# PatrickHwang/Explicit-tf2-Recommendation

Hardware: AMD Instinct MI355X
Metric: examples/sec fwd+bwd, DeepFM 10M-vocab x16d batch 8192 (higher is better)
Workload: dtype f32; 1 GPU; DeepFM fwd+bwd, 26 categorical fields, 10M-vocab x 16d, batch 8192 (BASELINE.json metric); vocab=10000000, fields=26, embedding_dims=16, batch_per_gpu=8192, id_distribution=uniform, parallelism=single GPU, global_batch=8192, hipgraph=one graph per 5 steps, 32 resident batches

## Files before the change

### explicit-tf2-recommendation_amd/csrc/deepfm_fused.hip

```cpp
#include "deepfm_fused.h"
#include <math.h>

namespace {

constexpr int LD = 32;

struct ReduceArgs {
  const float* dK0part; const float* small; int nwg; int D; int64_t B;
  float* dK0; float* dK1; float* db0; float* db1; float* dK2; float* db2; float* dbias; float* loss;
};

constexpr int RC = 16;
constexpr int RS = 64;
__host__ __device__ inline int reduce_blocks(int D) {
  return (int)(((int64_t)D * U1 / 4 + RC - 1) / RC) + (SMALL / 4 + RC - 1) / RC;
}

__device__ __forceinline__ void reduce_body(const ReduceArgs& r, int bidx) {
  const float* __restrict__ dK0part = r.dK0part;
  const float* __restrict__ small = r.small;
  const int nwg = r.nwg, D = r.D;
  const int64_t B = r.B;
  float* __restrict__ dK0 = r.dK0; float* __restrict__ dK1 = r.dK1; float* __restrict__ db0 = r.db0;
  float* __restrict__ db1 = r.db1; float* __restrict__ dK2 = r.dK2; float* __restrict__ db2 = r.db2;
  float* __restrict__ dbias = r.dbias; float* __restrict__ loss = r.loss;
  __shared__ float4 red[RS][RC];
  __shared__ float4 red2[8][RC];
  const int lane = threadIdx.x & (RC - 1), q = threadIdx.x / RC;
  const int64_t n0 = (int64_t)D * U1;
  const int nb0 = (int)((n0 / 4 + RC - 1) / RC);
  float4 acc = make_float4(0.f, 0.f, 0.f, 0.f);
  int64_t e4 = 0;
  const bool is_small = bidx >= nb0;
  const float* src;
  int64_t stride;
  bool in = false;
  if (!is_small) {
    e4 = (int64_t)bidx * RC + lane;
    in = e4 * 4 < n0;
    src = dK0part + e4 * 4;
    stride = n0;
  } else {
    e4 = (int64_t)(bidx - nb0) * RC + lane;
    in = e4 * 4 < SMALL;
    src = small + e4 * 4;
    stride = SMALL;
  }
  if (in) {
    int w = q;
    for (; w + 3 * RS < nwg; w += 4 * RS) {
      float4 x[4];
#pragma unroll
      for (int j = 0; j < 4; ++j) x[j] = *reinterpret_cast<const float4*>(src + (int64_t)(w + RS * j) * stride);
#pragma unroll
      for (int j = 0; j < 4; ++j) { acc.x += x[j].x; acc.y += x[j].y; acc.z += x[j].z; acc.w += x[j].w; }
    }
    for (; w < nwg; w += RS) {
      float4 x = *reinterpret_cast<const float4*>(src + (int64_t)w * stride);
      acc.x += x.x; acc.y += x.y; acc.z += x.z; acc.w += x.w;
    }
  }
  red[q][lane] = acc;
  __syncthreads();
  if (q < 8) {
    float4 s = red[8 * q][lane];
#pragma unroll
    for (int k = 1; k < 8; ++k) {
      float4 x = red[8 * q + k][lane];
      s.x += x.x; s.y += x.y; s.z += x.z; s.w += x.w;
    }
    red2[q][lane] = s;
  }
  __syncthreads();
  if (q != 0) return;
  float4 s = red2[0][lane];
#pragma unroll
  for (int k = 1; k < 8; ++k) {
    float4 x = red2[k][lane];
    s.x += x.x; s.y += x.y; s.z += x.z; s.w += x.w;
  }
  if (!is_small) {
    if (e4 * 4 < n0) *reinterpret_cast<float4*>(dK0 + e4 * 4) = s;
    return;
  }
  if (e4 * 4 >= SMALL) return;
  float sv[4] = {s.x, s.y, s.z, s.w};
#pragma unroll
  for (int i = 0; i < 4; ++i) {
    int k = (int)(e4 * 4) + i;
    if (k < SM_DB0) dK1[k - SM_DK1] = sv[i];
    else if (k < SM_DB1) db0[k - SM_DB0] = sv[i];
    else if (k < SM_DK2) db1[k - SM_DB1] = sv[i];
    else if (k < SM_DB2) dK2[k - SM_DK2] = sv[i];
    else if (k == SM_DB2) { db2[0] = sv[i]; dbias[0] = sv[i]; }
    else if (k == SM_LOSS) loss[0] = sv[i] / (float)B;
  }
}

struct ColSegArgs {
  const float4* vals; const float* gz; const int32_t* perm; const int64_t* col_uid; const int32_t* col_seg;
  const int32_t* col_nu; int64_t B; int F; int64_t* uniq_ids; float4* g_embed; float* g_w; int64_t* n_uniq; int packed;
  float* table; float* m_e; float* v_e; float* m_w; float* v_w; int64_t V; float lr_t, b1, b2, eps;
  const int32_t* slot_map;
  const float* lr_t_dev;
  int64_t ldm, ldw;
  int32_t* last; const int64_t* step_dev;
};

__device__ __forceinline__ void adam_chunk(const ColSegArgs& k, int64_t id, int c, const float4& g) {
  float4* vp = reinterpret_cast<float4*>(k.table + id * LD) + c;
  float4* mp = reinterpret_cast<float4*>(k.m_e + id * k.ldm) + c;
  float4* qp = reinterpret_cast<float4*>(k.v_e + id * k.ldm) + c;
  float4 x = *vp, m = *mp, v = *qp;
  adam_touch(x.x, m.x, v.x, g.x, k.lr_t, k.b1, k.b2, k.eps);
  adam_touch(x.y, m.y, v.y, g.y, k.lr_t, k.b1, k.b2, k.eps);
  adam_touch(x.z, m.z, v.z, g.z, k.lr_t, k.b1, k.b2, k.eps);
  adam_touch(x.w, m.w, v.w, g.w, k.lr_t, k.b1, k.b2, k.eps);
  *vp = x; *mp = m; *qp = v;
}
__device__ __forceinline__ void adam_w(const ColSegArgs& k, int64_t id, float g) {
  float x = k.table[id * LD + E16], m = k.m_w[id * k.ldw], v = k.v_w[id * k.ldw];
  adam_touch(x, m, v, g, k.lr_t, k.b1, k.b2, k.eps);
  k.table[id * LD + E16] = x; k.m_w[id * k.ldw] = m; k.v_w[id * k.ldw] = v;
}

__device__ __forceinline__ void colseg_body(const ColSegArgs& k, int bidx) {
  const float4* __restrict__ vals = k.vals;
  const float* __restrict__ gz = k.gz;
  const int32_t* __restrict__ perm = k.perm;
  const int64_t* __restrict__ col_uid = k.col_uid;
  const int32_t* __restrict__ col_seg = k.col_seg;
  const int32_t* __restrict__ col_nu = k.col_nu;
  const int64_t B = k.B;
  const int F = k.F;
  int64_t* __restrict__ uniq_ids = k.uniq_ids;
  float4* __restrict__ g_embed = k.g_embed;
  float* __restrict__ g_w = k.g_w;
  int64_t* __restrict__ n_uniq = k.n_uniq;
  const int packed = k.packed;
  const int tid = threadIdx.x, lane = tid & 63;
  const int c = tid & 3;
  const int64_t grp = ((int64_t)bidx * blockDim.x + tid) >> 2;
  const int f = (int)(grp / B);
  int u = (int)(grp - (int64_t)f * B);
  if ((B & 63) == 0) {
    const int w = u >> 4, g = u & 15;
    u = (g >> 2) * (int)(B >> 2) + 4 * w + (g & 3);
  }
  const bool in_range = f < F;
  __shared__ int nu_s[REC_MAX_COLS];
  if (tid < F) nu_s[tid] = col_nu[tid];
  __syncthreads();
  int64_t before = 0, total = 0;
  for (int q = 0; q < F; ++q) {
    int nq = nu_s[q];
    if (q < f) before += nq;
    total += nq;
  }
  const int nu = in_range ? nu_s[f] : 0;
  const bool live = in_range && u < nu;
  int s0 = 0, s1 = 0;
  if (live) {
    s0 = col_seg[(int64_t)f * (B + 1) + u];
    s1 = col_seg[(int64_t)f * (B + 1) + u + 1];
  }
  float4 acc = make_float4(0.f, 0.f, 0.f, 0.f);
  float accw = 0.f;
  const int32_t* pf = perm + (int64_t)f * B;
  int s_end = s1 < s0 + 16 ? s1 : s0 + 16;
  for (int s = s0; s < s_end; ++s) {
    int64_t b = pf[s];
    float4 x = vals[(b * F + f) * 4 + c];
    acc.x += x.x; acc.y += x.y; acc.z += x.z; acc.w += x.w;
    accw += gz[b];
  }
  unsigned long long longm = __ballot(live && (s1 - s0) > 16 && c == 0);
  while (longm) {
    int src = __ffsll((long long)longm) - 1;
    longm &= longm - 1;
    int rs0 = __shfl(s0, src, 64) + 16, rs1 = __shfl(s1, src, 64);
    int rf = __shfl(f, src, 64);
    const int32_t* rp = perm + (int64_t)rf * B;
    float4 pa = make_float4(0.f, 0.f, 0.f, 0.f);
    float pw = 0.f;
#pragma unroll 4
    for (int s = rs0 + (lane >> 2); s < rs1; s += 16) {
      int64_t b = rp[s];
      float4 x = vals[(b * F + rf) * 4 + c];
      pa.x += x.x; pa.y += x.y; pa.z += x.z; pa.w += x.w;
      pw += gz[b];
    }
#pragma unroll
    for (int o = 4; o < 64; o <<= 1) {
      pa.x += __shfl_xor(pa.x, o, 64); pa.y += __shfl_xor(pa.y, o, 64);
      pa.z += __shfl_xor(pa.z, o, 64); pa.w += __shfl_xor(pa.w, o, 64);
      pw += __shfl_xor(pw, o, 64);
    }
    if ((lane & ~3) == src) {
      acc.x += pa.x; acc.y += pa.y; acc.z += pa.z; acc.w += pa.w;
      accw += pw;
    }
  }
  if (!in_range) return;
  int64_t dst;
  int64_t idv;
  if (live) {
    dst = before + u;
    idv = col_uid[(int64_t)f * B + u];
    if (k.slot_map) dst = k.slot_map[dst];
  } else {
    if (k.slot_map) return;
    dst = total + ((int64_t)f * B - before) + (u - nu);
    idv = col_uid[0];
    acc = make_float4(0.f, 0.f, 0.f, 0.f);
    accw = 0.f;
  }
  if (packed) {
    g_embed[dst * 5 + c] = acc;
    if (c == 0) g_embed[dst * 5 + 4] = make_float4(accw, 0.f, 0.f, 0.f);
  } else {
    g_embed[dst * 4 + c] = acc;
    if (c == 0) g_w[dst] = accw;
  }
  if (c == 0 && uniq_ids) uniq_ids[dst] = idv;
  if (grp == 0 && c == 0 && n_uniq) *n_uniq = total;
}


constexpr int FIX_T = 1024, FIX_HUGE = 128, FIX_SHORT = 17, FIX_SKEW = 256;
__device__ __forceinline__ int fix_deal(int t, int64_t B) {
  if ((B & 63) != 0) return t;
  return ((t & 63) >> 2) * (int)(B >> 4) + 4 * (t >> 6) + (t & 3);
}
__device__ __forceinline__ int fix_spread(int t, int64_t B) {
  if ((B & 63) != 0) return t;
  return (t & 63) * (int)(B >> 6) + (t >> 6);
}
__device__ __forceinline__ int fix_group_src(unsigned long long mask, int lane) {
  int src = -1;
  const int g = lane >> 2;
  for (int i = 0; i < 16 && mask; ++i) {
    const int sl = __ffsll((long long)mask) - 1;
    mask &= mask - 1;
    if (g == i) src = sl;
  }
  return src;
}
__device__ __forceinline__ void fixup_body(const ColSegArgs& k_in, int bidx) {
  ColSegArgs k = k_in;
  if (k.lr_t_dev) k.lr_t = *k.lr_t_dev;
  const float4* __restrict__ vals = k.vals;
  const float* __restrict__ gz = k.gz;
  const int64_t B = k.B;
  const int F = k.F;
  float4* __restrict__ g_embed = k.g_embed;
  const int tid = threadIdx.x, lane = tid & 63;
  const int per_col = (int)((B + FIX_T - 1) / FIX_T);
  const int f = bidx / per_col;
  const int t = (bidx - f * per_col) * FIX_T + tid;
  const int u = fix_deal(t, B);
  __shared__ int nu_s[REC_MAX_COLS];
  __shared__ int huge_n, huge_s0[128], huge_s1[128], huge_u[128];
  __shared__ float huge_gz[128];
  __shared__ float4 hpart[FIX_T / 64][4];
  __shared__ float hw_s[FIX_T / 64];
  if (tid < F) nu_s[tid] = k.col_nu[tid];
  if (tid == 0) huge_n = 0;
  __syncthreads();
  int64_t before = 0, total = 0;
  for (int q = 0; q < F; ++q) {
    const int nq = nu_s[q];
    if (q < f) before += nq;
    total += nq;
  }
  const int nu = nu_s[f];
  const bool in_col = t < B;
  const bool live = in_col && u < nu;
  const int32_t* pf = k.perm + (int64_t)f * B;
  int s0 = 0, s1 = 0;
  if (live) {
    s0 = k.col_seg[(int64_t)f * (B + 1) + u];
    s1 = k.col_seg[(int64_t)f * (B + 1) + u + 1];
  }
  const int len = s1 - s0;
  const int64_t dst = before + u;
  const bool adam = k.table != nullptr;
  float accw = 0.f;
  if (live) {
    accw = gz[pf[s0]];
    const int64_t id = k.col_uid[(int64_t)f * B + u];
    if (len == 2) {
      const int64_t b2 = pf[s0 + 1];
      const float4* r2 = vals + (b2 * F + f) * 4;
      float4 a0 = g_embed[dst * 4], a1 = g_embed[dst * 4 + 1], a2 = g_embed[dst * 4 + 2], a3 = g_embed[dst * 4 + 3];
      const float4 x0 = r2[0], x1 = r2[1], x2 = r2[2], x3 = r2[3];
      a0.x += x0.x; a0.y += x0.y; a0.z += x0.z; a0.w += x0.w;
      a1.x += x1.x; a1.y += x1.y; a1.z += x1.z; a1.w += x1.w;
      a2.x += x2.x; a2.y += x2.y; a2.z += x2.z; a2.w += x2.w;
      a3.x += x3.x; a3.y += x3.y; a3.z += x3.z; a3.w += x3.w;
      g_embed[dst * 4] = a0; g_embed[dst * 4 + 1] = a1; g_embed[dst * 4 + 2] = a2; g_embed[dst * 4 + 3] = a3;
      k.g_w[dst] = accw + gz[b2];
    }
    if (len == 1) k.g_w[dst] = accw;
    k.uniq_ids[dst] = id;
  } else if (in_col) {
    const int64_t d2 = total + ((int64_t)f * B - before) + (u - nu);
    const float4 z = make_float4(0.f, 0.f, 0.f, 0.f);
    g_embed[d2 * 4] = z; g_embed[d2 * 4 + 1] = z; g_embed[d2 * 4 + 2] = z; g_embed[d2 * 4 + 3] = z;
    k.g_w[d2] = 0.f;
    k.uniq_ids[d2] = k.col_uid[0];
  }
  const bool skew = B - nu > FIX_SKEW;
  const int ub = skew ? fix_spread(t, B) : u;
  int s0b = s0, s1b = s1;
  if (skew) {
    s0b = 0; s1b = 0;
    if (in_col && ub < nu) {
      s0b = k.col_seg[(int64_t)f * (B + 1) + ub];
      s1b = k.col_seg[(int64_t)f * (B + 1) + ub + 1];
    }
  }
  const int lenb = s1b - s0b;
  float accwb = 0.f;
  if (lenb > 2) accwb = skew ? gz[pf[s0b]] : accw;
  if (skew && lenb > FIX_HUGE) {
    const int i = atomicAdd(&huge_n, 1);
    if (i < 128) { huge_s0[i] = s0b; huge_s1[i] = s1b; huge_u[i] = ub; huge_gz[i] = accwb; }
  }
  const int r = lane >> 2, c = lane & 3;
  {
    unsigned long long shortm = __ballot(skew && lenb > 2 && lenb <= FIX_SHORT);
#ifdef ABL_NOSHORT
    shortm = 0;
#endif
    while (shortm) {
      const int src = fix_group_src(shortm, lane);
      const bool has = src >= 0;
      const int sl = has ? src : 0;
      const int gs0 = __shfl(s0b, sl, 64), gs1_ = __shfl(s1b, sl, 64), gu = __shfl(ub, sl, 64);
      float wsum = __shfl(accwb, sl, 64);
      const int gs1 = has ? gs1_ : 0;
      const int64_t gdst = before + gu;
      float4 acc = make_float4(0.f, 0.f, 0.f, 0.f);
      if (has) acc = g_embed[gdst * 4 + c];
      for (int sp = gs0 + 1; __any(sp < gs1); sp += 4) {
        if (sp < gs1) {
          int e[4];
#pragma unroll
          for (int j = 0; j < 4; ++j) e[j] = pf[sp + j < gs1 ? sp + j : gs1 - 1];
          float4 xm[4];
          float gm[4];
#pragma unroll
          for (int j = 0; j < 4; ++j) {
            xm[j] = vals[((int64_t)e[j] * F + f) * 4 + c];
            gm[j] = gz[e[j]];
          }
#pragma unroll
          for (int j = 0; j < 4; ++j) {
            if (sp + j < gs1) {
              acc.x += xm[j].x; acc.y += xm[j].y; acc.z += xm[j].z; acc.w += xm[j].w;
              wsum += gm[j];
            }
          }
        }
      }
      if (has) {
        g_embed[gdst * 4 + c] = acc;
        if (c == 0) k.g_w[gdst] = wsum;
      }
      for (int i = 0; i < 16 && shortm; ++i) shortm &= shortm - 1;
    }
  }
  unsigned long long longm = __ballot(skew ? (lenb > FIX_SHORT && lenb <= FIX_HUGE) : lenb > 2);
#ifdef ABL_NOLONG
  longm = 0;
#endif
  while (longm) {
    const int src = __ffsll((long long)longm) - 1;
    longm &= longm - 1;
    const int rs0 = __shfl(s0b, src, 64), rs1 = __shfl(s1b, src, 64);
    const int ru = __shfl(ub, src, 64);
    const float rgz = __shfl(accwb, src, 64);
    const int64_t rdst = before + ru;
    float4 pa = make_float4(0.f, 0.f, 0.f, 0.f);
    float pw = 0.f;
#pragma unroll 4
    for (int s = rs0 + 1 + r; s < rs1; s += 16) {
      const int64_t b = pf[s];
      const float4 x = vals[(b * F + f) * 4 + c];
      pa.x += x.x; pa.y += x.y; pa.z += x.z; pa.w += x.w;
      pw += gz[b];
    }
#pragma unroll
    for (int o = 4; o < 64; o <<= 1) {
      pa.x += __shfl_xor(pa.x, o, 64); pa.y += __shfl_xor(pa.y, o, 64);
      pa.z += __shfl_xor(pa.z, o, 64); pa.w += __shfl_xor(pa.w, o, 64);
      pw += __shfl_xor(pw, o, 64);
    }
    if (r == 0) {
      float4 h = g_embed[rdst * 4 + c];
      h.x += pa.x; h.y += pa.y; h.z += pa.z; h.w += pa.w;
      g_embed[rdst * 4 + c] = h;
      const float wsum = rgz + pw;
      if (c == 0) k.g_w[rdst] = wsum;
    }
  }
  if (skew) __syncthreads();
#ifdef ABL_NOHUGE
  const int n_huge = 0;
#else
  const int n_huge = skew ? (huge_n < 128 ? huge_n : 128) : 0;
#endif
  const int wv = tid >> 6;
  constexpr int NWV_F = FIX_T / 64;
  if (n_huge > NWV_F) {
    int hs0 = 0, hs1 = 0, hu = 0, rk = 0;
    float hg = 0.f;
    if (tid < n_huge) {
      hs0 = huge_s0[tid]; hs1 = huge_s1[tid]; hu = huge_u[tid]; hg = huge_gz[tid];
      for (int j = 0; j < n_huge; ++j) rk += huge_u[j] < hu ? 1 : 0;
    }
    __syncthreads();
    if (tid < n_huge) { huge_s0[rk] = hs0; huge_s1[rk] = hs1; huge_u[rk] = hu; huge_gz[rk] = hg; }
    __syncthreads();
  }
  for (int h0 = 0; h0 < n_huge; h0 += NWV_F) {
    const int nr = n_huge - h0 < NWV_F ? n_huge - h0 : NWV_F;
    const int wpr = NWV_F / nr;
    const int hl = wv / wpr, sw = wv - hl * wpr;
    const bool mine = hl < nr;
    const int h = h0 + (mine ? hl : 0);
    const int rs0 = huge_s0[h], rs1 = mine ? huge_s1[h] : 0;
    float4 pa = make_float4(0.f, 0.f, 0.f, 0.f);
    float pw = 0.f;
    const int stride = 16 * wpr;
    for (int base = rs0 + 1 + 16 * sw + r; base < rs1; base += 4 * stride) {
      int bm[4];
#pragma unroll
      for (int j = 0; j < 4; ++j) {
        const int sidx = base + j * stride;
        bm[j] = pf[sidx < rs1 ? sidx : rs1 - 1];
      }
      float4 xm[4];
      float gm[4];
#pragma unroll
      for (int j = 0; j < 4; ++j) {
        xm[j] = vals[((int64_t)bm[j] * F + f) * 4 + c];
        gm[j] = gz[bm[j]];
      }
#pragma unroll
      for (int j = 0; j < 4; ++j) {
        if (base + j * stride < rs1) {
          pa.x += xm[j].x; pa.y += xm[j].y; pa.z += xm[j].z; pa.w += xm[j].w;
          pw += gm[j];
        }
      }
    }
#pragma unroll
    for (int o = 4; o < 64; o <<= 1) {
      pa.x += __shfl_xor(pa.x, o, 64); pa.y += __shfl_xor(pa.y, o, 64);
      pa.z += __shfl_xor(pa.z, o, 64); pa.w += __shfl_xor(pa.w, o, 64);
      pw += __shfl_xor(pw, o, 64);
    }
    float4 hsum = make_float4(0.f, 0.f, 0.f, 0.f);
    const int64_t rdst = before + huge_u[h];
    const bool fin = mine && sw == 0 && r == 0;
    if (fin) hsum = g_embed[rdst * 4 + c];
    if (r == 0) {
      hpart[wv][c] = pa;
      if (c == 0) hw_s[wv] = pw;
    }
    __syncthreads();
    if (fin) {
      float wsum = huge_gz[h];
      for (int q = 0; q < wpr; ++q) {
        const float4 x = hpart[wv + q][c];
        hsum.x += x.x; hsum.y += x.y; hsum.z += x.z; hsum.w += x.w;
        wsum += hw_s[wv + q];
      }
      g_embed[rdst * 4 + c] = hsum;
      if (c == 0) k.g_w[rdst] = wsum;
    }
    __syncthreads();
  }
  if (bidx == 0 && tid == 0) *k.n_uniq = total;
  if (adam) {
    __syncthreads();
    const int piece = tid & 7, rr = tid >> 3;
    const int step_now = k.last ? (int32_t)*k.step_dev : 0;
    const bool skew_a = B - nu > FIX_SKEW;
#pragma unroll 1
    for (int p = 0; p < (skew_a ? 2 : 1) * (FIX_T / 128); ++p) {
      const bool spread = p >= FIX_T / 128;
      const int tl = (bidx - f * per_col) * FIX_T + (spread ? p - FIX_T / 128 : p) * 128 + rr;
      const int uu = spread ? fix_spread(tl, B) : fix_deal(tl, B);
      if (tl < B && uu < nu && piece < 5) {
        const int ln = k.col_seg[(int64_t)f * (B + 1) + uu + 1] - k.col_seg[(int64_t)f * (B + 1) + uu];
        if (!skew_a || (ln > 2) == spread) {
          const int64_t d2 = before + uu;
          const int64_t id = k.col_uid[(int64_t)f * B + uu];
          if ((uint64_t)id < (uint64_t)k.V) {
            if (piece < 4) {
              adam_chunk(k, id, piece, g_embed[d2 * 4 + piece]);
            } else {
              adam_w(k, id, k.g_w[d2]);
              if (k.last) k.last[id] = step_now;
            }
          }
        }
      }
    }
  }
}

__global__ __launch_bounds__(1024, 8) void deepfm_post_direct_kernel(ReduceArgs r, ColSegArgs k, int nb_reduce) {
  if ((int)blockIdx.x < nb_reduce) reduce_body(r, (int)blockIdx.x);
  else fixup_body(k, (int)blockIdx.x - nb_reduce);
}

__global__ __launch_bounds__(1024) void deepfm_post_kernel(ReduceArgs r, ColSegArgs k, int nb_reduce) {
  if ((int)blockIdx.x < nb_reduce) reduce_body(r, (int)blockIdx.x);
  else colseg_body(k, (int)blockIdx.x - nb_reduce);
}


struct CatchArgs {
  const int64_t* col_uid; const int32_t* col_nu; int64_t B; int F;
  float* table; int64_t V; float* m_e; float* v_e; int64_t ldm; float* m_w; float* v_w; int64_t ldw;
  const int32_t* last; const int64_t* step_dev; const float* lr_tab; int64_t n_tab; float b1, b2, eps;
};
constexpr int CATCH_R = 64, CATCH_T = 256, CATCH_LR = 1024;
__global__ __launch_bounds__(CATCH_T) void adam_keras_catchup_kernel(CatchArgs a) {
  __shared__ float4 x_s[CATCH_R][4], m_s[CATCH_R][4], v_s[CATCH_R][4];
  __shared__ float xw_s[CATCH_R], mw_s[CATCH_R], vw_s[CATCH_R];
  __shared__ int64_t id_s[CATCH_R];
  __shared__ int k_s[CATCH_R];
  __shared__ unsigned char ord[CATCH_R];
  __shared__ float lr_s[CATCH_LR];
  const int tid = threadIdx.x, r = tid >> 2, q = tid & 3;
  const int64_t nslot = a.col_uid ? a.B * a.F : a.V;
  const int64_t j1 = *a.step_dev;
#pragma unroll
  for (int i = tid; i < CATCH_LR; i += CATCH_T) {
    const int64_t j = j1 - i;
    lr_s[i] = j >= 1 ? a.lr_tab[(j < a.n_tab ? j : a.n_tab) - 1] : 0.f;
  }
  const int64_t slot = (int64_t)blockIdx.x * CATCH_R + r;
  int64_t id = -1;
  if (a.col_uid) {
    const int64_t sc = slot < nslot ? slot : nslot - 1;
    const int f = (int)(sc / a.B);
    const int64_t u = sc - (int64_t)f * a.B;
    const int nu = a.col_nu[f];
    const int64_t cand = a.col_uid[sc];
    if (slot < nslot && u < nu) id = cand;
  } else if (slot < nslot) {
    id = slot;
  }
  const bool ok = (uint64_t)id < (uint64_t)a.V;
  const int64_t idc = ok ? id : 0;
  const int j0 = a.last[idc];
  float4 x4 = *reinterpret_cast<const float4*>(a.table + idc * LD + 4 * q);
  float4 m4 = *reinterpret_cast<const float4*>(a.m_e + idc * a.ldm + 4 * q);
  float4 v4 = *reinterpret_cast<const float4*>(a.v_e + idc * a.ldm + 4 * q);
  x_s[r][q] = x4; m_s[r][q] = m4; v_s[r][q] = v4;
  if (q == 0) {
    xw_s[r] = a.table[idc * LD + E16];
    mw_s[r] = a.m_w[idc * a.ldw];
    vw_s[r] = a.v_w[idc * a.ldw];
    id_s[r] = id;
    k_s[r] = (ok && j1 > j0) ? (int)(j1 - j0) : 0;
  }
  __syncthreads();
  if (tid < CATCH_R) {
    const int k = k_s[tid];
    int rank = 0;
#pragma unroll 8
    for (int c = 0; c < CATCH_R; ++c) rank += (k_s[c] > k || (k_s[c] == k && c < tid)) ? 1 : 0;
    ord[rank] = (unsigned char)tid;
  }
  __syncthreads();
  const int rr = ord[r];
  const int k = k_s[rr];
  if (k <= 0) return;
  const int64_t rid = id_s[rr];
  x4 = x_s[rr][q]; m4 = m_s[rr][q]; v4 = v_s[rr][q];
  float xw = 0.f, mw = 0.f, vw = 0.f;
  if (q == 0) { xw = xw_s[rr]; mw = mw_s[rr]; vw = vw_s[rr]; }
  const bool any_e = m4.x != 0.f || v4.x != 0.f || m4.y != 0.f || v4.y != 0.f || m4.z != 0.f || v4.z != 0.f ||
                     m4.w != 0.f || v4.w != 0.f;
  const bool any_w = q == 0 && (mw != 0.f || vw != 0.f);
  if (!any_e && !any_w) return;
  for (int i = k - 1; i >= 0; --i) {
    float lr;
    if (i < CATCH_LR) {
      lr = lr_s[i];
    } else {
      const int64_t j = j1 - i;
      lr = a.lr_tab[(j < a.n_tab ? j : a.n_tab) - 1];
    }
    adam_decay(x4.x, m4.x, v4.x, lr, a.b1, a.b2, a.eps);
    adam_decay(x4.y, m4.y, v4.y, lr, a.b1, a.b2, a.eps);
    adam_decay(x4.z, m4.z, v4.z, lr, a.b1, a.b2, a.eps);
    adam_decay(x4.w, m4.w, v4.w, lr, a.b1, a.b2, a.eps);
    if (q == 0) adam_decay(xw, mw, vw, lr, a.b1, a.b2, a.eps);
  }
  if (any_e) {
    *reinterpret_cast<float4*>(a.table + rid * LD + 4 * q) = x4;
    *reinterpret_cast<float4*>(a.m_e + rid * a.ldm + 4 * q) = m4;
    *reinterpret_cast<float4*>(a.v_e + rid * a.ldm + 4 * q) = v4;
  }
  if (any_w) {
    a.table[rid * LD + E16] = xw;
    a.m_w[rid * a.ldw] = mw;
    a.v_w[rid * a.ldw] = vw;
  }
}
__global__ __launch_bounds__(256) void fill_last_kernel(int32_t* __restrict__ last, int64_t V,
                                                        const int64_t* __restrict__ step_dev) {
  const int64_t t = (int64_t)blockIdx.x * 256 + threadIdx.x;
  if (t < V) last[t] = (int32_t)*step_dev;
}

}

extern "C" size_t rec_deepfm_fused_workspace_bytes(int64_t B, int F) {
  if (B <= 0 || F <= 0) return 0;
  return fused_workspace(B, F).bytes() + 256;
}

extern "C" int rec_deepfm_fused_post_f32(int F, int64_t B, const float* gz, const float* vals, float* const* grads,
                                         float* loss, void* workspace, const int32_t* perm, const int64_t* col_uid,
                                         const int32_t* col_seg, const int32_t* col_nu, int64_t* uniq_ids,
                                         float* g_embed_rows, float* g_w_rows, int64_t* n_uniq, const int32_t* slot_map,
                                         int direct, const rec_deepfm_lazy_adam* adam, void* stream) {
  if (adam) {
    if (!adam->table || !adam->m_e || !adam->v_e || !adam->m_w || !adam->v_w || !adam->lr_t_dev || adam->V <= 0 ||
        adam->ld_state < E16 || (adam->ld_state & 3) != 0 || adam->ld_wstate < 1)
      return REC_E_ARG;
    if (adam->ld != LD || !rec_is_aligned16(adam->table) || !rec_is_aligned16(adam->m_e) || !rec_is_aligned16(adam->v_e))
      return REC_E_UNSUPPORTED;
    if (adam->last && !adam->step_dev) return REC_E_ARG;
  }
  if (B <= 0 || F <= 0 || F > 28) return REC_E_ARG;
  if (!gz || !vals || !grads || !loss || !workspace || !perm || !col_uid || !col_seg || !col_nu || !g_embed_rows)
    return REC_E_ARG;
  for (int i = 0; i < 7; ++i)
    if (!grads[i]) return REC_E_ARG;
  if (slot_map ? (uniq_ids || g_w_rows || n_uniq) : (!uniq_ids || !g_w_rows || !n_uniq)) return REC_E_ARG;
  if ((slot_map && direct) || (adam && !direct)) return REC_E_UNSUPPORTED;
  if (!rec_is_aligned16(vals) || !rec_is_aligned16(g_embed_rows))
    return REC_E_UNSUPPORTED;
  const FusedWorkspace ws = fused_workspace(B, F);
  int D = F * E16;
  unsigned nb = (unsigned)reduce_blocks(D);
  ReduceArgs r{ws.dK0part(workspace), ws.small(workspace), ws.nwg, D, B,
               grads[0], grads[2], grads[1], grads[3], grads[4], grads[5], grads[6], loss};
  ColSegArgs k{};
  k.vals = (const float4*)vals; k.gz = gz; k.perm = perm; k.col_uid = col_uid; k.col_seg = col_seg; k.col_nu = col_nu;
  k.B = B; k.F = F; k.uniq_ids = uniq_ids; k.g_embed = (float4*)g_embed_rows; k.g_w = g_w_rows; k.n_uniq = n_uniq;
  k.packed = slot_map ? 1 : 0; k.slot_map = slot_map;
  if (adam) {
    k.table = adam->table; k.m_e = adam->m_e; k.v_e = adam->v_e; k.m_w = adam->m_w; k.v_w = adam->v_w; k.V = adam->V;
    k.b1 = adam->b1; k.b2 = adam->b2; k.eps = adam->eps; k.lr_t_dev = adam->lr_t_dev;
    k.ldm = adam->ld_state; k.ldw = adam->ld_wstate; k.last = adam->last; k.step_dev = adam->step_dev;
  }
  if (direct) {
    unsigned nbf = (unsigned)F * (unsigned)ceil_div64(B, FIX_T);
    hipLaunchKernelGGL(deepfm_post_direct_kernel, dim3(nb + nbf), dim3(1024), 0, as_stream(stream), r, k, (int)nb);
  } else {
    unsigned nbs = (unsigned)ceil_div64(B * F * 4, 1024);
    hipLaunchKernelGGL(deepfm_post_kernel, dim3(nb + nbs), dim3(1024), 0, as_stream(stream), r, k, (int)nb);
  }
  REC_LAUNCH_CHECK();
  return REC_OK;
}

static int catchup_args_ok(const float* table, int64_t ld, int64_t V, const float* m_e, const float* v_e, int64_t ld_state,
                           const float* m_w, const float* v_w, int64_t ld_wstate, const int32_t* last,
                           const int64_t* step_dev, const float* lr_table, int64_t n_table) {
  if (!table || !m_e || !v_e || !m_w || !v_w || !last || !step_dev || !lr_table || V <= 0 || n_table <= 0 ||
      ld_state < E16 || ld_wstate < 1)
    return REC_E_ARG;
  if (ld != LD) return REC_E_UNSUPPORTED;
  if ((ld_state & 3) != 0 || !rec_is_aligned16(table) || !rec_is_aligned16(m_e) || !rec_is_aligned16(v_e))
    return REC_E_UNSUPPORTED;
  return REC_OK;
}

extern "C" int rec_adam_keras_catchup_f32(const int64_t* col_uid, const int32_t* col_nu, int64_t B, int F, float* table,
                                          int64_t ld, int64_t V, float* m_e, float* v_e, int64_t ld_state, float* m_w,
                                          float* v_w, int64_t ld_wstate, const int32_t* last, const int64_t* step_dev,
                                          const float* lr_table, int64_t n_table, float b1, float b2, float eps,
                                          void* stream) {
  if (!col_uid || !col_nu || B <= 0 || F <= 0) return REC_E_ARG;
  int rc = catchup_args_ok(table, ld, V, m_e, v_e, ld_state, m_w, v_w, ld_wstate, last, step_dev, lr_table, n_table);
  if (rc != REC_OK) return rc;
  CatchArgs a{col_uid, col_nu, B, F, table, V, m_e, v_e, ld_state, m_w, v_w, ld_wstate, last, step_dev, lr_table, n_table,
              b1, b2, eps};
  hipLaunchKernelGGL(adam_keras_catchup_kernel, dim3((unsigned)ceil_div64(B * F, CATCH_R)), dim3(CATCH_T), 0,
                     as_stream(stream), a);
  REC_LAUNCH_CHECK();
  return REC_OK;
}

extern "C" int rec_adam_keras_flush_f32(float* table, int64_t ld, int64_t V, float* m_e, float* v_e, int64_t ld_state,
                                        float* m_w, float* v_w, int64_t ld_wstate, int32_t* last, const int64_t* step_dev,
                                        const float* lr_table, int64_t n_table, float b1, float b2, float eps,
                                        void* stream) {
  int rc = catchup_args_ok(table, ld, V, m_e, v_e, ld_state, m_w, v_w, ld_wstate, last, step_dev, lr_table, n_table);
  if (rc != REC_OK) return rc;
  CatchArgs a{nullptr, nullptr, 0, 0, table, V, m_e, v_e, ld_state, m_w, v_w, ld_wstate, last, step_dev, lr_table,
              n_table, b1, b2, eps};
  hipLaunchKernelGGL(adam_keras_catchup_kernel, dim3((unsigned)ceil_div64(V, CATCH_R)), dim3(CATCH_T), 0,
                     as_stream(stream), a);
  REC_LAUNCH_CHECK();
  hipLaunchKernelGGL(fill_last_kernel, dim3((unsigned)ceil_div64(V, 256)), dim3(256), 0, as_stream(stream), last, V,
                     step_dev);
  REC_LAUNCH_CHECK();
  return REC_OK;
}
```

Baseline: 247.4 million examples/s.

## Add quad-per-lane fixup path in direct post kernel with helper waves

Adds a new fixup body for the direct post kernel, used when there is no lazy Adam and B is a multiple of FIX_T. Each lane of the first waves handles four consecutive unique rows with vectorized segment/id loads and vector stores, and a second group of waves processes long runs in parallel. Column offsets are computed with a wave prefix scan instead of shared memory plus a serial loop, and 32-bit indexing replaces 64-bit (guarded by a size check). Fixup blocks are now scheduled before reduce blocks, and optional timestamp instrumentation is compiled in only under a debug macro. The aim is more memory-level parallelism per thread and less index and sync overhead, at the cost of more branching and code complexity.

```diff
diff --git a/explicit-tf2-recommendation_amd/csrc/deepfm_fused.hip b/explicit-tf2-recommendation_amd/csrc/deepfm_fused.hip
--- a/explicit-tf2-recommendation_amd/csrc/deepfm_fused.hip
+++ b/explicit-tf2-recommendation_amd/csrc/deepfm_fused.hip
@@ -4,10 +4,31 @@
 namespace {
 
 constexpr int LD = 32;
+
+#ifdef REC_POST_STAMPS
+#define PSTAMP_WG(wg_) const int pstamp_wg = (wg_)
+#define PSTAMP(A, k_)                                                                                          \
+  do {                                                                                                         \
+    if ((threadIdx.x & 63) == 0)                                                                               \
+      (A).stamps[((int64_t)pstamp_wg * 16 + (threadIdx.x >> 6)) * 8 + (k_)] = wall_clock64();                  \
+  } while (0)
+#ifdef REC_POST_STAMPS_NOWAIT
+#define PSTAMP_WAIT() do {} while (0)
+#else
+#define PSTAMP_WAIT() asm volatile("s_waitcnt vmcnt(0)" ::: "memory")
+#endif
+#else
+#define PSTAMP_WG(wg_) do {} while (0)
+#define PSTAMP(A, k_) do {} while (0)
+#define PSTAMP_WAIT() do {} while (0)
+#endif
 
 struct ReduceArgs {
   const float* dK0part; const float* small; int nwg; int D; int64_t B;
   float* dK0; float* dK1; float* db0; float* db1; float* dK2; float* db2; float* dbias; float* loss;
+#ifdef REC_POST_STAMPS
+  unsigned long long* stamps;
+#endif
 };
 
 constexpr int RC = 16;
@@ -27,6 +48,8 @@
   __shared__ float4 red[RS][RC];
   __shared__ float4 red2[8][RC];
   const int lane = threadIdx.x & (RC - 1), q = threadIdx.x / RC;
+  PSTAMP_WG(bidx);
+  PSTAMP(r, 0);
   const int64_t n0 = (int64_t)D * U1;
   const int nb0 = (int)((n0 / 4 + RC - 1) / RC);
   float4 acc = make_float4(0.f, 0.f, 0.f, 0.f);
@@ -60,8 +83,11 @@
       acc.x += x.x; acc.y += x.y; acc.z += x.z; acc.w += x.w;
     }
   }
+  PSTAMP_WAIT();
+  PSTAMP(r, 1);
   red[q][lane] = acc;
   __syncthreads();
+  PSTAMP(r, 2);
   if (q < 8) {
     float4 s = red[8 * q][lane];
 #pragma unroll
@@ -81,6 +107,7 @@
   }
   if (!is_small) {
     if (e4 * 4 < n0) *reinterpret_cast<float4*>(dK0 + e4 * 4) = s;
+    PSTAMP(r, 3);
     return;
   }
   if (e4 * 4 >= SMALL) return;
@@ -95,6 +122,7 @@
     else if (k == SM_DB2) { db2[0] = sv[i]; dbias[0] = sv[i]; }
     else if (k == SM_LOSS) loss[0] = sv[i] / (float)B;
   }
+  PSTAMP(r, 3);
 }
 
 struct ColSegArgs {
@@ -105,6 +133,9 @@
   const float* lr_t_dev;
   int64_t ldm, ldw;
   int32_t* last; const int64_t* step_dev;
+#ifdef REC_POST_STAMPS
+  unsigned long long* stamps;
+#endif
 };
 
 __device__ __forceinline__ void adam_chunk(const ColSegArgs& k, int64_t id, int c, const float4& g) {
@@ -246,90 +277,83 @@
   }
   return src;
 }
-__device__ __forceinline__ void fixup_body(const ColSegArgs& k_in, int bidx) {
-  ColSegArgs k = k_in;
-  if (k.lr_t_dev) k.lr_t = *k.lr_t_dev;
+struct FixShared {
+  int huge_n, huge_s0[128], huge_s1[128], huge_u[128];
+  float huge_gz[128];
+  float4 hpart[FIX_T / 64][4];
+  float hw_s[FIX_T / 64];
+};
+
+template <typename IX, bool HEADGZ = false>
+__device__ __forceinline__ void fix_wave_runs(const ColSegArgs& k, const int32_t* __restrict__ pf, int f, IX before,
+                                              unsigned long long longm, int s0b, int s1b, int ub, float accwb) {
   const float4* __restrict__ vals = k.vals;
   const float* __restrict__ gz = k.gz;
+  float4* __restrict__ g_embed = k.g_embed;
+  const int F = k.F;
+  const int lane = threadIdx.x & 63, r = lane >> 2, c = lane & 3;
+#ifdef ABL_NOLONG
+  longm = 0;
+#endif
+  while (longm) {
+    const int src = __ffsll((long long)longm) - 1;
+    longm &= longm - 1;
+    const int rs0 = __shfl(s0b, src, 64), rs1 = __shfl(s1b, src, 64);
+    const int ru = __shfl(ub, src, 64);
+    float rgz = __shfl(accwb, src, 64);
+    const IX rdst = before + ru;
+    float4 h = make_float4(0.f, 0.f, 0.f, 0.f);
+    if (r == 0) h = g_embed[rdst * 4 + c];
+    if (HEADGZ) rgz = gz[pf[rs0]];
+    float4 pa = make_float4(0.f, 0.f, 0.f, 0.f);
+    float pw = 0.f;
+#pragma unroll 4
+    for (int s = rs0 + 1 + r; s < rs1; s += 16) {
+      const IX b = pf[s];
+      const float4 x = vals[(b * F + f) * 4 + c];
+      pa.x += x.x; pa.y += x.y; pa.z += x.z; pa.w += x.w;
+      pw += gz[b];
+    }
+#pragma unroll
+    for (int o = 4; o < 64; o <<= 1) {
+      pa.x += __shfl_xor(pa.x, o, 64); pa.y += __shfl_xor(pa.y, o, 64);
+      pa.z += __shfl_xor(pa.z, o, 64); pa.w += __shfl_xor(pa.w, o, 64);
+      pw += __shfl_xor(pw, o, 64);
+    }
+    if (r == 0) {
+      h.x += pa.x; h.y += pa.y; h.z += pa.z; h.w += pa.w;
+      g_embed[rdst * 4 + c] = h;
+      const float wsum = rgz + pw;
+      if (c == 0) k.g_w[rdst] = wsum;
+    }
+  }
+}
+
+template <typename IX>
+__device__ __forceinline__ void fix_skew_runs(const ColSegArgs& k, FixShared& sh, const int32_t* __restrict__ pf, int f,
+                                              IX before, int nu, bool in_col, int t) {
+  const float4* __restrict__ vals = k.vals;
+  const float* __restrict__ gz = k.gz;
+  float4* __restrict__ g_embed = k.g_embed;
   const int64_t B = k.B;
   const int F = k.F;
-  float4* __restrict__ g_embed = k.g_embed;
   const int tid = threadIdx.x, lane = tid & 63;
-  const int per_col = (int)((B + FIX_T - 1) / FIX_T);
-  const int f = bidx / per_col;
-  const int t = (bidx - f * per_col) * FIX_T + tid;
-  const int u = fix_deal(t, B);
-  __shared__ int nu_s[REC_MAX_COLS];
-  __shared__ int huge_n, huge_s0[128], huge_s1[128], huge_u[128];
-  __shared__ float huge_gz[128];
-  __shared__ float4 hpart[FIX_T / 64][4];
-  __shared__ float hw_s[FIX_T / 64];
-  if (tid < F) nu_s[tid] = k.col_nu[tid];
-  if (tid == 0) huge_n = 0;
-  __syncthreads();
-  int64_t before = 0, total = 0;
-  for (int q = 0; q < F; ++q) {
-    const int nq = nu_s[q];
-    if (q < f) before += nq;
-    total += nq;
-  }
-  const int nu = nu_s[f];
-  const bool in_col = t < B;
-  const bool live = in_col && u < nu;
-  const int32_t* pf = k.perm + (int64_t)f * B;
-  int s0 = 0, s1 = 0;
-  if (live) {
-    s0 = k.col_seg[(int64_t)f * (B + 1) + u];
-    s1 = k.col_seg[(int64_t)f * (B + 1) + u + 1];
-  }
-  const int len = s1 - s0;
-  const int64_t dst = before + u;
-  const bool adam = k.table != nullptr;
-  float accw = 0.f;
-  if (live) {
-    accw = gz[pf[s0]];
-    const int64_t id = k.col_uid[(int64_t)f * B + u];
-    if (len == 2) {
-      const int64_t b2 = pf[s0 + 1];
-      const float4* r2 = vals + (b2 * F + f) * 4;
-      float4 a0 = g_embed[dst * 4], a1 = g_embed[dst * 4 + 1], a2 = g_embed[dst * 4 + 2], a3 = g_embed[dst * 4 + 3];
-      const float4 x0 = r2[0], x1 = r2[1], x2 = r2[2], x3 = r2[3];
-      a0.x += x0.x; a0.y += x0.y; a0.z += x0.z; a0.w += x0.w;
-      a1.x += x1.x; a1.y += x1.y; a1.z += x1.z; a1.w += x1.w;
-      a2.x += x2.x; a2.y += x2.y; a2.z += x2.z; a2.w += x2.w;
-      a3.x += x3.x; a3.y += x3.y; a3.z += x3.z; a3.w += x3.w;
-      g_embed[dst * 4] = a0; g_embed[dst * 4 + 1] = a1; g_embed[dst * 4 + 2] = a2; g_embed[dst * 4 + 3] = a3;
-      k.g_w[dst] = accw + gz[b2];
-    }
-    if (len == 1) k.g_w[dst] = accw;
-    k.uniq_ids[dst] = id;
-  } else if (in_col) {
-    const int64_t d2 = total + ((int64_t)f * B - before) + (u - nu);
-    const float4 z = make_float4(0.f, 0.f, 0.f, 0.f);
-    g_embed[d2 * 4] = z; g_embed[d2 * 4 + 1] = z; g_embed[d2 * 4 + 2] = z; g_embed[d2 * 4 + 3] = z;
-    k.g_w[d2] = 0.f;
-    k.uniq_ids[d2] = k.col_uid[0];
-  }
-  const bool skew = B - nu > FIX_SKEW;
-  const int ub = skew ? fix_spread(t, B) : u;
-  int s0b = s0, s1b = s1;
-  if (skew) {
-    s0b = 0; s1b = 0;
-    if (in_col && ub < nu) {
-      s0b = k.col_seg[(int64_t)f * (B + 1) + ub];
-      s1b = k.col_seg[(int64_t)f * (B + 1) + ub + 1];
-    }
+  const int ub = fix_spread(t, B);
+  int s0b = 0, s1b = 0;
+  if (in_col && ub < nu) {
+    s0b = k.col_seg[(IX)f * (IX)(B + 1) + ub];
+    s1b = k.col_seg[(IX)f * (IX)(B + 1) + ub + 1];
   }
   const int lenb = s1b - s0b;
   float accwb = 0.f;
-  if (lenb > 2) accwb = skew ? gz[pf[s0b]] : accw;
-  if (skew && lenb > FIX_HUGE) {
-    const int i = atomicAdd(&huge_n, 1);
-    if (i < 128) { huge_s0[i] = s0b; huge_s1[i] = s1b; huge_u[i] = ub; huge_gz[i] = accwb; }
+  if (lenb > 2) accwb = gz[pf[s0b]];
+  if (lenb > FIX_HUGE) {
+    const int i = atomicAdd(&sh.huge_n, 1);
+    if (i < 128) { sh.huge_s0[i] = s0b; sh.huge_s1[i] = s1b; sh.huge_u[i] = ub; sh.huge_gz[i] = accwb; }
   }
   const int r = lane >> 2, c = lane & 3;
   {
-    unsigned long long shortm = __ballot(skew && lenb > 2 && lenb <= FIX_SHORT);
+    unsigned long long shortm = __ballot(lenb > 2 && lenb <= FIX_SHORT);
 #ifdef ABL_NOSHORT
     shortm = 0;
 #endif
@@ -340,7 +364,7 @@
       const int gs0 = __shfl(s0b, sl, 64), gs1_ = __shfl(s1b, sl, 64), gu = __shfl(ub, sl, 64);
       float wsum = __shfl(accwb, sl, 64);
       const int gs1 = has ? gs1_ : 0;
-      const int64_t gdst = before + gu;
+      const IX gdst = before + gu;
       float4 acc = make_float4(0.f, 0.f, 0.f, 0.f);
       if (has) acc = g_embed[gdst * 4 + c];
       for (int sp = gs0 + 1; __any(sp < gs1); sp += 4) {
@@ -352,7 +376,7 @@
           float gm[4];
 #pragma unroll
           for (int j = 0; j < 4; ++j) {
-            xm[j] = vals[((int64_t)e[j] * F + f) * 4 + c];
+            xm[j] = vals[((IX)e[j] * F + f) * 4 + c];
             gm[j] = gz[e[j]];
           }
 #pragma unroll
@@ -371,45 +395,12 @@
       for (int i = 0; i < 16 && shortm; ++i) shortm &= shortm - 1;
     }
   }
-  unsigned long long longm = __ballot(skew ? (lenb > FIX_SHORT && lenb <= FIX_HUGE) : lenb > 2);
-#ifdef ABL_NOLONG
-  longm = 0;
-#endif
-  while (longm) {
-    const int src = __ffsll((long long)longm) - 1;
-    longm &= longm - 1;
-    const int rs0 = __shfl(s0b, src, 64), rs1 = __shfl(s1b, src, 64);
-    const int ru = __shfl(ub, src, 64);
-    const float rgz = __shfl(accwb, src, 64);
-    const int64_t rdst = before + ru;
-    float4 pa = make_float4(0.f, 0.f, 0.f, 0.f);
-    float pw = 0.f;
-#pragma unroll 4
-    for (int s = rs0 + 1 + r; s < rs1; s += 16) {
-      const int64_t b = pf[s];
-      const float4 x = vals[(b * F + f) * 4 + c];
-      pa.x += x.x; pa.y += x.y; pa.z += x.z; pa.w += x.w;
-      pw += gz[b];
-    }
-#pragma unroll
-    for (int o = 4; o < 64; o <<= 1) {
-      pa.x += __shfl_xor(pa.x, o, 64); pa.y += __shfl_xor(pa.y, o, 64);
-      pa.z += __shfl_xor(pa.z, o, 64); pa.w += __shfl_xor(pa.w, o, 64);
-      pw += __shfl_xor(pw, o, 64);
-    }
-    if (r == 0) {
-      float4 h = g_embed[rdst * 4 + c];
-      h.x += pa.x; h.y += pa.y; h.z += pa.z; h.w += pa.w;
-      g_embed[rdst * 4 + c] = h;
-      const float wsum = rgz + pw;
-      if (c == 0) k.g_w[rdst] = wsum;
-    }
-  }
-  if (skew) __syncthreads();
+  fix_wave_runs<IX>(k, pf, f, before, __ballot(lenb > FIX_SHORT && lenb <= FIX_HUGE), s0b, s1b, ub, accwb);
+  __syncthreads();
 #ifdef ABL_NOHUGE
   const int n_huge = 0;
 #else
-  const int n_huge = skew ? (huge_n < 128 ? huge_n : 128) : 0;
+  const int n_huge = sh.huge_n < 128 ? sh.huge_n : 128;
 #endif
   const int wv = tid >> 6;
   constexpr int NWV_F = FIX_T / 64;
@@ -417,11 +408,11 @@
     int hs0 = 0, hs1 = 0, hu = 0, rk = 0;
     float hg = 0.f;
     if (tid < n_huge) {
-      hs0 = huge_s0[tid]; hs1 = huge_s1[tid]; hu = huge_u[tid]; hg = huge_gz[tid];
-      for (int j = 0; j < n_huge; ++j) rk += huge_u[j] < hu ? 1 : 0;
+      hs0 = sh.huge_s0[tid]; hs1 = sh.huge_s1[tid]; hu = sh.huge_u[tid]; hg = sh.huge_gz[tid];
+      for (int j = 0; j < n_huge; ++j) rk += sh.huge_u[j] < hu ? 1 : 0;
     }
     __syncthreads();
-    if (tid < n_huge) { huge_s0[rk] = hs0; huge_s1[rk] = hs1; huge_u[rk] = hu; huge_gz[rk] = hg; }
+    if (tid < n_huge) { sh.huge_s0[rk] = hs0; sh.huge_s1[rk] = hs1; sh.huge_u[rk] = hu; sh.huge_gz[rk] = hg; }
     __syncthreads();
   }
   for (int h0 = 0; h0 < n_huge; h0 += NWV_F) {
@@ -430,7 +421,7 @@
     const int hl = wv / wpr, sw = wv - hl * wpr;
     const bool mine = hl < nr;
     const int h = h0 + (mine ? hl : 0);
-    const int rs0 = huge_s0[h], rs1 = mine ? huge_s1[h] : 0;
+    const int rs0 = sh.huge_s0[h], rs1 = mine ? sh.huge_s1[h] : 0;
     float4 pa = make_float4(0.f, 0.f, 0.f, 0.f);
     float pw = 0.f;
     const int stride = 16 * wpr;
@@ -445,7 +436,7 @@
       float gm[4];
 #pragma unroll
       for (int j = 0; j < 4; ++j) {
-        xm[j] = vals[((int64_t)bm[j] * F + f) * 4 + c];
+        xm[j] = vals[((IX)bm[j] * F + f) * 4 + c];
         gm[j] = gz[bm[j]];
       }
 #pragma unroll
@@ -463,26 +454,103 @@
       pw += __shfl_xor(pw, o, 64);
     }
     float4 hsum = make_float4(0.f, 0.f, 0.f, 0.f);
-    const int64_t rdst = before + huge_u[h];
+    const IX rdst = before + sh.huge_u[h];
     const bool fin = mine && sw == 0 && r == 0;
     if (fin) hsum = g_embed[rdst * 4 + c];
     if (r == 0) {
-      hpart[wv][c] = pa;
-      if (c == 0) hw_s[wv] = pw;
+      sh.hpart[wv][c] = pa;
+      if (c == 0) sh.hw_s[wv] = pw;
     }
     __syncthreads();
     if (fin) {
-      float wsum = huge_gz[h];
+      float wsum = sh.huge_gz[h];
       for (int q = 0; q < wpr; ++q) {
-        const float4 x = hpart[wv + q][c];
+        const float4 x = sh.hpart[wv + q][c];
         hsum.x += x.x; hsum.y += x.y; hsum.z += x.z; hsum.w += x.w;
-        wsum += hw_s[wv + q];
+        wsum += sh.hw_s[wv + q];
       }
       g_embed[rdst * 4 + c] = hsum;
       if (c == 0) k.g_w[rdst] = wsum;
     }
     __syncthreads();
   }
+}
+
+__device__ __forceinline__ void fixup_body(const ColSegArgs& k_in, int bidx) {
+  ColSegArgs k = k_in;
+  if (k.lr_t_dev) k.lr_t = *k.lr_t_dev;
+  const float4* __restrict__ vals = k.vals;
+  const float* __restrict__ gz = k.gz;
+  const int64_t B = k.B;
+  const int F = k.F;
+  float4* __restrict__ g_embed = k.g_embed;
+  const int tid = threadIdx.x;
+  const int per_col = (int)((B + FIX_T - 1) / FIX_T);
+  PSTAMP_WG((int)gridDim.x - F * per_col + bidx);
+  PSTAMP(k, 0);
+  const int f = bidx / per_col;
+  const int t = (bidx - f * per_col) * FIX_T + tid;
+  const int u = fix_deal(t, B);
+  __shared__ int nu_s[REC_MAX_COLS];
+  __shared__ FixShared sh;
+  if (tid < F) nu_s[tid] = k.col_nu[tid];
+  if (tid == 0) sh.huge_n = 0;
+  __syncthreads();
+  PSTAMP(k, 1);
+  int64_t before = 0, total = 0;
+  for (int q = 0; q < F; ++q) {
+    const int nq = nu_s[q];
+    if (q < f) before += nq;
+    total += nq;
+  }
+  const int nu = nu_s[f];
+  const bool in_col = t < B;
+  const bool live = in_col && u < nu;
+  const int32_t* pf = k.perm + (int64_t)f * B;
+  int s0 = 0, s1 = 0;
+  if (live) {
+    s0 = k.col_seg[(int64_t)f * (B + 1) + u];
+    s1 = k.col_seg[(int64_t)f * (B + 1) + u + 1];
+  }
+  const int len = s1 - s0;
+  const int64_t dst = before + u;
+  const bool adam = k.table != nullptr;
+  float accw = 0.f;
+  if (live) {
+    PSTAMP_WAIT();
+    PSTAMP(k, 2);
+    const int hb = pf[s0];
+    PSTAMP_WAIT();
+    PSTAMP(k, 3);
+    accw = gz[hb];
+    const int64_t id = k.col_uid[(int64_t)f * B + u];
+    PSTAMP_WAIT();
+    PSTAMP(k, 4);
+    if (len == 2) {
+      const int64_t b2 = pf[s0 + 1];
+      const float4* r2 = vals + (b2 * F + f) * 4;
+      float4 a0 = g_embed[dst * 4], a1 = g_embed[dst * 4 + 1], a2 = g_embed[dst * 4 + 2], a3 = g_embed[dst * 4 + 3];
+      const float4 x0 = r2[0], x1 = r2[1], x2 = r2[2], x3 = r2[3];
+      a0.x += x0.x; a0.y += x0.y; a0.z += x0.z; a0.w += x0.w;
+      a1.x += x1.x; a1.y += x1.y; a1.z += x1.z; a1.w += x1.w;
+      a2.x += x2.x; a2.y += x2.y; a2.z += x2.z; a2.w += x2.w;
+      a3.x += x3.x; a3.y += x3.y; a3.z += x3.z; a3.w += x3.w;
+      g_embed[dst * 4] = a0; g_embed[dst * 4 + 1] = a1; g_embed[dst * 4 + 2] = a2; g_embed[dst * 4 + 3] = a3;
+      k.g_w[dst] = accw + gz[b2];
+    }
+    if (len == 1) k.g_w[dst] = accw;
+    k.uniq_ids[dst] = id;
+  } else if (in_col) {
+    const int64_t d2 = total + ((int64_t)f * B - before) + (u - nu);
+    const float4 z = make_float4(0.f, 0.f, 0.f, 0.f);
+    g_embed[d2 * 4] = z; g_embed[d2 * 4 + 1] = z; g_embed[d2 * 4 + 2] = z; g_embed[d2 * 4 + 3] = z;
+    k.g_w[d2] = 0.f;
+    k.uniq_ids[d2] = k.col_uid[0];
+  }
+  PSTAMP(k, 5);
+  const bool skew = B - nu > FIX_SKEW;
+  if (skew) fix_skew_runs<int64_t>(k, sh, pf, f, before, nu, in_col, t);
+  else fix_wave_runs<int64_t>(k, pf, f, before, __ballot(len > 2), s0, s1, u, accw);
   if (bidx == 0 && tid == 0) *k.n_uniq = total;
   if (adam) {
     __syncthreads();
@@ -511,9 +579,168 @@
       }
     }
   }
-}
-
+  PSTAMP(k, 6);
+}
+
+constexpr int FIXQ_WV = FIX_T / 256;
+typedef int32_t fixq_seg4 __attribute__((ext_vector_type(4), aligned(4)));
+typedef long long fixq_id2 __attribute__((ext_vector_type(2)));
+__device__ __forceinline__ void fixq_body(const ColSegArgs& k, int bidx) {
+  const float4* __restrict__ vals = k.vals;
+  const float* __restrict__ gz = k.gz;
+  float4* __restrict__ g_embed = k.g_embed;
+  const int B = (int)k.B, F = k.F;
+  const int tid = threadIdx.x, lane = tid & 63;
+  const int wv = __builtin_amdgcn_readfirstlane(tid >> 6);
+  const int per_col = B >> 10;
+  PSTAMP_WG((int)gridDim.x - F * per_col + bidx);
+  PSTAMP(k, 0);
+  const int f = bidx / per_col;
+  const int wgc = bidx - f * per_col;
+  const bool fast = wv < FIXQ_WV;
+  const bool helper = !fast && wv < 2 * FIXQ_WV;
+  const int u0 = wgc * FIX_T + (fast || helper ? 256 * (wv & (FIXQ_WV - 1)) + 4 * lane : 0);
+  __shared__ FixShared sh;
+  const int nu_l = k.col_nu[lane < F ? lane : 0];
+  fixq_seg4 sg4 = {0, 0, 0, 0};
+  int sg4e = 0;
+  fixq_id2 id01 = {0, 0}, id23 = {0, 0};
+  int64_t id_pad = 0;
+  if (fast || helper) {
+    const int32_t* segp = k.col_seg + (f * (B + 1) + u0);
+    sg4 = *reinterpret_cast<const fixq_seg4*>(segp);
+    sg4e = segp[4];
+  }
+  if (fast) {
+    const fixq_id2* idp = reinterpret_cast<const fixq_id2*>(k.col_uid + (f * B + u0));
+    id01 = idp[0];
+    id23 = idp[1];
+    id_pad = k.col_uid[0];
+  }
+  int incl = lane < F ? nu_l : 0;
+#pragma unroll
+  for (int o = 1; o < 32; o <<= 1) {
+    const int x = __shfl_up(incl, o, 64);
+    if (lane >= o) incl += x;
+  }
+  const int before = __builtin_amdgcn_readlane(incl - (lane < F ? nu_l : 0), f);
+  const int total = __builtin_amdgcn_readlane(incl, F - 1);
+  const int nu = __builtin_amdgcn_readlane(nu_l, f);
+  PSTAMP(k, 1);
+  const bool skew = B - nu > FIX_SKEW;
+  const int32_t* pf = k.perm + f * B;
+  if (fast) {
+    const int nl = nu - u0;
+    const int sg[5] = {sg4.x, sg4.y, sg4.z, sg4.w, sg4e};
+    PSTAMP_WAIT();
+    PSTAMP(k, 2);
+    {
+    const int dst = before + u0;
+    if (nl >= 4) {
+      if ((dst & 1) == 0) {
+        fixq_id2* op = reinterpret_cast<fixq_id2*>(k.uniq_ids + dst);
+        op[0] = id01;
+        op[1] = id23;
+      } else {
+        k.uniq_ids[dst] = id01.x; k.uniq_ids[dst + 1] = id01.y; k.uniq_ids[dst + 2] = id23.x; k.uniq_ids[dst + 3] = id23.y;
+      }
+    } else {
+      const int64_t idv[4] = {id01.x, id01.y, id23.x, id23.y};
+      const int d2 = total + (f * B - before) + (u0 - nu);
+      const float4 z = make_float4(0.f, 0.f, 0.f, 0.f);
+      if (nl <= 0 && (d2 & 3) == 0) {
+#pragma unroll
+        for (int i = 0; i < 16; ++i) g_embed[d2 * 4 + i] = z;
+        *reinterpret_cast<float4*>(k.g_w + d2) = z;
+        const fixq_id2 p2 = {id_pad, id_pad};
+        fixq_id2* op = reinterpret_cast<fixq_id2*>(k.uniq_ids + d2);
+        op[0] = p2;
+        op[1] = p2;
+      } else {
+#pragma unroll
+        for (int j = 0; j < 4; ++j) {
+          if (j < nl) {
+            k.uniq_ids[dst + j] = idv[j];
+          } else {
+            g_embed[(d2 + j) * 4] = z; g_embed[(d2 + j) * 4 + 1] = z; g_embed[(d2 + j) * 4 + 2] = z;
+            g_embed[(d2 + j) * 4 + 3] = z;
+            k.g_w[d2 + j] = 0.f;
+            k.uniq_ids[d2 + j] = id_pad;
+          }
+        }
+      }
+    }
+    }
+    int ln[4], hb[4], hb2[4];
+#pragma unroll
+    for (int j = 0; j < 4; ++j) ln[j] = j < nl ? sg[j + 1] - sg[j] : 0;
+#pragma unroll
+    for (int j = 0; j < 4; ++j) hb[j] = pf[j < nl ? sg[j] : 0];
+#pragma unroll
+    for (int j = 0; j < 4; ++j) hb2[j] = pf[j < nl ? sg[j] + (ln[j] > 1 ? 1 : 0) : 0];
+    PSTAMP_WAIT();
+    PSTAMP(k, 3);
+    float gw[4];
+#pragma unroll
+    for (int j = 0; j < 4; ++j) gw[j] = gz[hb[j]];
+    asm volatile("" : "+v"(hb2[0]), "+v"(hb2[1]), "+v"(hb2[2]), "+v"(hb2[3]));
+    PSTAMP_WAIT();
+    PSTAMP(k, 4);
+    const int dst = before + u0;
+    const bool anylong = ln[0] > 2 || ln[1] > 2 || ln[2] > 2 || ln[3] > 2;
+    unsigned pm = (ln[0] == 2 ? 1u : 0u) | (ln[1] == 2 ? 2u : 0u) | (ln[2] == 2 ? 4u : 0u) | (ln[3] == 2 ? 8u : 0u);
+    while (pm) {
+      const int j = __ffs((int)pm) - 1;
+      pm &= pm - 1;
+      const int b2 = j == 0 ? hb2[0] : j == 1 ? hb2[1] : j == 2 ? hb2[2] : hb2[3];
+      const float4* r2 = vals + (b2 * F + f) * 4;
+      float4* hr = g_embed + (dst + j) * 4;
+      float4 a0 = hr[0], a1 = hr[1], a2 = hr[2], a3 = hr[3];
+      const float4 x0 = r2[0], x1 = r2[1], x2 = r2[2], x3 = r2[3];
+      const float g2 = gz[b2];
+      a0.x += x0.x; a0.y += x0.y; a0.z += x0.z; a0.w += x0.w;
+      a1.x += x1.x; a1.y += x1.y; a1.z += x1.z; a1.w += x1.w;
+      a2.x += x2.x; a2.y += x2.y; a2.z += x2.z; a2.w += x2.w;
+      a3.x += x3.x; a3.y += x3.y; a3.z += x3.z; a3.w += x3.w;
+      hr[0] = a0; hr[1] = a1; hr[2] = a2; hr[3] = a3;
+#pragma unroll
+      for (int i = 0; i < 4; ++i) gw[i] = i == j ? gw[i] + g2 : gw[i];
+    }
+    if (nl >= 4 && !anylong && (dst & 3) == 0) {
+      *reinterpret_cast<float4*>(k.g_w + dst) = make_float4(gw[0], gw[1], gw[2], gw[3]);
+    } else {
+#pragma unroll
+      for (int j = 0; j < 4; ++j)
+        if (ln[j] == 1 || ln[j] == 2) k.g_w[dst + j] = gw[j];
+    }
+    PSTAMP(k, 5);
+  }
+  if (helper && !skew) {
+    const int nl = nu - u0;
+    const int sg[5] = {sg4.x, sg4.y, sg4.z, sg4.w, sg4e};
+    PSTAMP_WAIT();
+    PSTAMP(k, 2);
+#pragma unroll
+    for (int j = 0; j < 4; ++j)
+      fix_wave_runs<int, true>(k, pf, f, before, __ballot(j < nl && sg[j + 1] - sg[j] > 2), sg[j], sg[j + 1], u0 + j, 0.f);
+  }
+  if (bidx == 0 && tid == 0) *k.n_uniq = total;
+  if (skew) {
+    if (tid == 0) sh.huge_n = 0;
+    __syncthreads();
+    fix_skew_runs<int>(k, sh, pf, f, before, nu, true, wgc * FIX_T + tid);
+  }
+  PSTAMP(k, 6);
+}
+
+template <bool QUADS>
 __global__ __launch_bounds__(1024, 8) void deepfm_post_direct_kernel(ReduceArgs r, ColSegArgs k, int nb_reduce) {
+  if (QUADS) {
+    const int nbf = (int)gridDim.x - nb_reduce;
+    if ((int)blockIdx.x < nbf) fixq_body(k, (int)blockIdx.x);
+    else reduce_body(r, (int)blockIdx.x - nbf);
+    return;
+  }
   if ((int)blockIdx.x < nb_reduce) reduce_body(r, (int)blockIdx.x);
   else fixup_body(k, (int)blockIdx.x - nb_reduce);
 }
@@ -624,6 +851,15 @@
 
 }
 
+#ifdef REC_POST_STAMPS
+static unsigned long long* g_post_stamps = nullptr;
+constexpr size_t POST_STAMP_WGS = 4096;
+extern "C" int rec_debug_post_stamps(unsigned long long* host_out, int n_wg) {
+  if (!g_post_stamps || n_wg < 0 || (size_t)n_wg > POST_STAMP_WGS) return REC_E_ARG;
+  return (int)hipMemcpy(host_out, g_post_stamps, sizeof(unsigned long long) * 8 * 16 * (size_t)n_wg, hipMemcpyDeviceToHost);
+}
+#endif
+
 extern "C" size_t rec_deepfm_fused_workspace_bytes(int64_t B, int F) {
   if (B <= 0 || F <= 0) return 0;
   return fused_workspace(B, F).bytes() + 256;
@@ -651,6 +887,7 @@
   if ((slot_map && direct) || (adam && !direct)) return REC_E_UNSUPPORTED;
   if (!rec_is_aligned16(vals) || !rec_is_aligned16(g_embed_rows))
     return REC_E_UNSUPPORTED;
+  if (B > (((int64_t)1 << 31) - 1) / ((int64_t)F * E16)) return REC_E_UNSUPPORTED;
   const FusedWorkspace ws = fused_workspace(B, F);
   int D = F * E16;
   unsigned nb = (unsigned)reduce_blocks(D);
@@ -667,7 +904,24 @@
   }
   if (direct) {
     unsigned nbf = (unsigned)F * (unsigned)ceil_div64(B, FIX_T);
-    hipLaunchKernelGGL(deepfm_post_direct_kernel, dim3(nb + nbf), dim3(1024), 0, as_stream(stream), r, k, (int)nb);
+#ifdef REC_POST_STAMPS
+    if (nb + nbf > POST_STAMP_WGS) return REC_E_UNSUPPORTED;
+    if (!g_post_stamps &&
+        (hipMalloc(&g_post_stamps, sizeof(unsigned long long) * 8 * 16 * POST_STAMP_WGS) != hipSuccess ||
+         hipMemset(g_post_stamps, 0, sizeof(unsigned long long) * 8 * 16 * POST_STAMP_WGS) != hipSuccess))
+      return REC_E_ARG;
+    r.stamps = g_post_stamps;
+    k.stamps = g_post_stamps;
+#endif
+    bool quads = !adam && (B % FIX_T) == 0 && rec_is_aligned16(col_uid) && rec_is_aligned16(uniq_ids) &&
+                 rec_is_aligned16(g_w_rows);
+#ifdef REC_POST_NO_QUADS
+    quads = false;
+#endif
+    if (quads)
+      hipLaunchKernelGGL(deepfm_post_direct_kernel<true>, dim3(nb + nbf), dim3(1024), 0, as_stream(stream), r, k, (int)nb);
+    else
+      hipLaunchKernelGGL(deepfm_post_direct_kernel<false>, dim3(nb + nbf), dim3(1024), 0, as_stream(stream), r, k, (int)nb);
   } else {
     unsigned nbs = (unsigned)ceil_div64(B * F * 4, 1024);
     hipLaunchKernelGGL(deepfm_post_kernel, dim3(nb + nbs), dim3(1024), 0, as_stream(stream), r, k, (int)nb);
```

New measurement: 269.4 million examples/s, median of 6. +8.9%, better.
